# Toytiny/CMFlow

Hardware: AMD Instinct MI355X
Metric: frame-pairs/sec CMFlow fwd+bwd (higher is better)
Workload: dtype f32; 1 GPU; cmflow fwd+bwd training (7 cross-modal losses + Adam, train-mode BN) step, N=256, B=64 per GPU (global 64), ball-query r=2/4/8/16 K=4/8/16/32, kNN K=8; synthetic clouds, seeded random-init weights; parallelism=dp1

## Files before the change

cmflow_amd/csrc/gemm.hip:

```cpp
#include <algorithm>
#include <atomic>
#include <cstdlib>
#include <cstring>
#include <type_traits>
#include "cmf_common.h"
#include "../../include/cmflow_hip.h"

typedef float f32x16 __attribute__((ext_vector_type(16)));

constexpr int G_THREADS = 256;
#ifndef CMF_GEMM_BK
#define CMF_GEMM_BK 16
#endif
constexpr int G_BK = CMF_GEMM_BK;
constexpr int G_KT = G_BK / 4;
constexpr int G_RP = 256 / G_KT;
constexpr int G_LDS_LD = G_BK + 4;

#include "gemm_args.h"
#ifdef CMF_GEMM_DIAG
#define GDIAG(p) ((p).diag)
#else
#define GDIAG(p) 0
#endif
// ... 45 lines not shown
}

template <int BM, int BN, bool A_T, bool B_T, int EPI = 0, int GMODE = 0>
__global__ __launch_bounds__(G_THREADS, (BM > 128 || BN > 128) ? 2 : 3) void gemm_kernel(const GemmArgs p)
{
    constexpr bool GATHER = GMODE == 1, GATHER_B = GMODE == 2, GATHER_Z = GMODE == 3 || GMODE == 4, GATHER_S = GMODE == 4;
    static_assert(!GATHER_Z || (!A_T && !B_T && EPI == 4 && (BM == 128 || (BM == 256 && GMODE == 4)) && BN == 128), "gathered Z rows: the kind-4 data gradient");
    static_assert(!GATHER || (!A_T && B_T), "gathering A operand: A[M][K] W[N][K] layout");
    static_assert(!GATHER_B || (A_T && !B_T), "gathering B operand: A[K][M] B[K][N] layout");
    constexpr int WARPS_M = (BM == 64) ? 2 : ((BN >= 128) ? 2 : 4);
    constexpr int WARPS_N = 4 / WARPS_M;
    constexpr int WM = BM / WARPS_M, WN = BN / WARPS_N;
    constexpr int TM = WM / 32, TN = WN / 32;
    static_assert(TM >= 1 && TN >= 1, "tile");
    constexpr int A_LD = A_T ? BM + 4 : G_LDS_LD, A_SZ = A_T ? G_BK * (BM + 4) : BM * G_LDS_LD;
    constexpr int B_LD = B_T ? G_LDS_LD : BN + 4, B_SZ = B_T ? BN * G_LDS_LD : G_BK * (BN + 4);
    extern __shared__ __attribute__((aligned(16))) float smem[];
    float *As = smem;
    float *Bs = smem + 2 * A_SZ;

    const int tiles_m = (p.M + BM - 1) / BM, tiles_n = (p.N + BN - 1) / BN;
    int tm, tn, split;
    {
        const int id = blockIdx.x, nx = 8;
        const int xcd = id % nx, slot = id / nx;
        if (p.split_k > 1) {
            const int tiles = tiles_m * tiles_n;
            split = xcd + nx * (slot / tiles);
            const int t = slot % tiles;
            tm = t / tiles_n; tn = t % tiles_n;
            if (split >= p.split_k) return;
        } else {
            const int per = (tiles_m + nx - 1) / nx;
            split = 0;
            tm = xcd * per + slot / tiles_n;
            tn = slot % tiles_n;
            if (tm >= tiles_m || slot / tiles_n >= per) return;
        }
    }
    const unsigned long long t_start = p.trace ? wall_clock64() : 0ull;
    const int kchunks_total = (p.K + G_BK - 1) / G_BK;
    const int kchunks_per = (kchunks_total + p.split_k - 1) / p.split_k;
    const int kc_begin = split * kchunks_per;
    const int kc_end = min(kchunks_total, kc_begin + kchunks_per);
    const int m0 = tm * BM, n0 = tn * BN;
    const int tid = threadIdx.x, lane = tid & 63, wid = __builtin_amdgcn_readfirstlane(tid >> 6);
    const int wm = wid / WARPS_N, wn = wid % WARPS_N;

    constexpr int A_TPR = BM / 4, A_RPI = G_THREADS / A_TPR;
    constexpr int B_TPR = BN / 4, B_RPI = G_THREADS / B_TPR;
    constexpr int A_IT = A_T ? (G_BK / A_RPI) : (BM / G_RP);
    constexpr int B_IT = B_T ? (BN / G_RP) : (G_BK / B_RPI);
    float4 ra[A_IT], rb[B_IT];
    int gbrow[GATHER_B ? B_IT : 1];
    float4 gbd[GATHER_B ? B_IT : 1], gbw[3];
    float4 rz[A_T ? A_IT : 1];
    const bool bnbA = A_T && p.bnb_z != nullptr;
    float bal[4] = {1.f, 1.f, 1.f, 1.f}, bbe[4] = {0.f, 0.f, 0.f, 0.f}, bga[4] = {0.f, 0.f, 0.f, 0.f}, bmu[4] = {0.f, 0.f, 0.f, 0.f};
    int k0_loaded = 0;
    const int bnb_writers = tiles_n < G_BK ? tiles_n : G_BK;
    if (A_T && bnbA) {
        const int m = m0 + (tid % A_TPR) * 4;
#pragma unroll
        for (int j = 0; j < 4; ++j) {
            bmu[j] = p.bnb_mean[m + j];
            cmf_bnb_coef(p.bnb_a[m + j], bmu[j], p.bnb_invstd[m + j], p.bnb_sums[m + j], p.bnb_sums[p.M + m + j], p.bnb_ic,
                         bal[j], bbe[j], bga[j]);
        }
    }
    float4 psa = make_float4(1.f, 1.f, 1.f, 1.f), psc = make_float4(0.f, 0.f, 0.f, 0.f);
    float4 qsa = make_float4(1.f, 1.f, 1.f, 1.f), qsc = make_float4(0.f, 0.f, 0.f, 0.f);
    unsigned kmask = 0xF;
    const bool proA = !A_T && p.pro_a != nullptr;
    const bool proB = !B_T && p.prob_a != nullptr;
    const bool edge_mn = (m0 + BM > p.M) || (n0 + BN > p.N);
    if (proB) {
        const int n = n0 + (tid % B_TPR) * 4;
        float t[8] = {1, 1, 1, 1, 0, 0, 0, 0};
        for (int j = 0; j < 4; ++j) if (n + j < p.N) { t[j] = p.prob_a[n + j]; t[4 + j] = p.prob_c[n + j]; }
        qsa = make_float4(t[0], t[1], t[2], t[3]); qsc = make_float4(t[4], t[5], t[6], t[7]);
    }

    auto load_tiles = [&](int kc) {
        const int k0 = kc * G_BK;
        const bool fast = !edge_mn && (k0 + G_BK <= p.K);
        k0_loaded = k0;
        if (fast) {
            if (!A_T) {
                const int kk = k0 + (tid % G_KT) * 4;
                if (proA) { psa = *(const float4 *)(p.pro_a + kk); psc = *(const float4 *)(p.pro_c + kk); }
                const float *src = p.A + (long long)(m0 + (tid / G_KT)) * p.lda + kk;
#pragma unroll
                for (int i = 0; i < A_IT; ++i) ra[i] = *(const float4 *)(src + (long long)G_RP * i * p.lda);
            } else {
                const float *src = p.A + (long long)(k0 + tid / A_TPR) * p.lda + m0 + (tid % A_TPR) * 4;
#pragma unroll
                for (int i = 0; i < A_IT; ++i) ra[i] = *(const float4 *)(src + (long long)A_RPI * i * p.lda);
                if (bnbA) {
                    const float *zs = p.bnb_z + (long long)(k0 + tid / A_TPR) * p.ldbz + m0 + (tid % A_TPR) * 4;
#pragma unroll
                    for (int i = 0; i < A_IT; ++i) rz[A_T ? i : 0] = *(const float4 *)(zs + (long long)A_RPI * i * p.ldbz);
                }
            }
            if (B_T) {
                const float *src = p.B + (long long)(n0 + (tid / G_KT)) * p.ldb + k0 + (tid % G_KT) * 4;
#pragma unroll
                for (int i = 0; i < B_IT; ++i) rb[i] = *(const float4 *)(src + (long long)G_RP * i * p.ldb);
            } else if (GATHER_B) {
#pragma unroll
                for (int i = 0; i < B_IT; ++i) {
                    const int k = k0 + tid / B_TPR + B_RPI * i;
                    rb[GATHER_B ? i : 0] = *(const float4 *)(p.B + (long long)gbrow[GATHER_B ? i : 0] * p.ldb + n0 + (tid % B_TPR) * 4);
                    gbd[GATHER_B ? i : 0] = *(const float4 *)(p.ga_dxyz + (long long)k * 4);
                    gbrow[GATHER_B ? i : 0] = k + G_BK < p.K ? p.ga_rows[k + G_BK] : 0;
                }
            } else {
                const float *src = p.B + (long long)(k0 + tid / B_TPR) * p.ldb + n0 + (tid % B_TPR) * 4;
#pragma unroll
                for (int i = 0; i < B_IT; ++i) rb[i] = *(const float4 *)(src + (long long)B_RPI * i * p.ldb);
            }
            kmask = 0xF;
            return;
        }
        if (GATHER_B) __builtin_trap();
        auto ld4 = [&](const float *src, int valid) {
            float t[4] = {0.f, 0.f, 0.f, 0.f};
            if (valid >= 4) return *(const float4 *)src;
            for (int j = 0; j < 4; ++j) if (j < valid) t[j] = src[j];
            return make_float4(t[0], t[1], t[2], t[3]);
        };
        if (!A_T) {
            const int kk = k0 + (tid % G_KT) * 4;
            const int kv = max(0, min(4, p.K - kk));
            kmask = (1u << kv) - 1u;
            if (proA) { psa = ld4(p.pro_a + kk, kv); psc = ld4(p.pro_c + kk, kv); }
#pragma unroll
            for (int i = 0; i < A_IT; ++i) {
                const int m = m0 + (tid / G_KT) + G_RP * i;
                ra[i] = (m < p.M && kv > 0) ? ld4(p.A + (long long)m * p.lda + kk, kv) : make_float4(0.f, 0.f, 0.f, 0.f);
                if (m >= p.M) ra[i].x = __builtin_nanf("");
            }
        } else {
#pragma unroll
            for (int i = 0; i < A_IT; ++i) {
                const int k = k0 + tid / A_TPR + A_RPI * i, m = m0 + (tid % A_TPR) * 4;
                ra[i] = (k < p.K && m < p.M) ? ld4(p.A + (long long)k * p.lda + m, p.M - m) : make_float4(0.f, 0.f, 0.f, 0.f);
            }
        }
        if (B_T) {
            const int kk = k0 + (tid % G_KT) * 4;
            const int kv = max(0, min(4, p.K - kk));
#pragma unroll
            for (int i = 0; i < B_IT; ++i) {
                const int n = n0 + (tid / G_KT) + G_RP * i;
                rb[i] = (n < p.N && kv > 0) ? ld4(p.B + (long long)n * p.ldb + kk, kv) : make_float4(0.f, 0.f, 0.f, 0.f);
            }
        } else {
#pragma unroll
            for (int i = 0; i < B_IT; ++i) {
                const int k = k0 + tid / B_TPR + B_RPI * i, n = n0 + (tid % B_TPR) * 4;
                rb[i] = (k < p.K && n < p.N) ? ld4(p.B + (long long)k * p.ldb + n, p.N - n) : make_float4(0.f, 0.f, 0.f, 0.f);
                if (!(k < p.K)) rb[i].x = __builtin_nanf("");
            }
        }
    };
    auto pro4 = [&](float4 v, const float4 &sa, const float4 &sc) {
        v.x = fmaxf(fmaf(sa.x, v.x, sc.x), 0.f); v.y = fmaxf(fmaf(sa.y, v.y, sc.y), 0.f);
        v.z = fmaxf(fmaf(sa.z, v.z, sc.z), 0.f); v.w = fmaxf(fmaf(sa.w, v.w, sc.w), 0.f);
        return v;
    };
    auto store_A = [&](int buf) {
        float *dst = As + buf * A_SZ;
        if (!A_T) {
#pragma unroll
            for (int i = 0; i < A_IT; ++i) {
                float4 v = ra[i];
                if (proA) {
                    const bool dead = v.x != v.x;
                    v = pro4(v, psa, psc);
                    if (dead) v = make_float4(0.f, 0.f, 0.f, 0.f);
                    if (kmask != 0xF) { if (!(kmask & 1)) v.x = 0.f; if (!(kmask & 2)) v.y = 0.f;
                                        if (!(kmask & 4)) v.z = 0.f; if (!(kmask & 8)) v.w = 0.f; }
                } else if (v.x != v.x && edge_mn) v = make_float4(0.f, 0.f, 0.f, 0.f);
                *(float4 *)(dst + ((tid / G_KT) + G_RP * i) * G_LDS_LD + (tid % G_KT) * 4) = v;
            }
        } else {
#pragma unroll
            for (int i = 0; i < A_IT; ++i) {
                const int k = tid / A_TPR + A_RPI * i, m = (tid % A_TPR) * 4;
                float4 v = ra[i];
                if (bnbA) {
                    const float4 zz = rz[A_T ? i : 0];
                    v.x = cmf_bnb_apply(v.x, zz.x, bmu[0], bal[0], bbe[0], bga[0]); v.y = cmf_bnb_apply(v.y, zz.y, bmu[1], bal[1], bbe[1], bga[1]);
                    v.z = cmf_bnb_apply(v.z, zz.z, bmu[2], bal[2], bbe[2], bga[2]); v.w = cmf_bnb_apply(v.w, zz.w, bmu[3], bal[3], bbe[3], bga[3]);
                    if (p.bnb_out && (k % bnb_writers) == tn) *(float4 *)(p.bnb_out + (long long)(k0_loaded + k) * p.ldbo + m0 + m) = v;
                }
                *(float4 *)(dst + k * A_LD + m) = v;
            }
        }
    };
    auto store_B = [&](int buf) {
        float *dst = Bs + buf * B_SZ;
        if (B_T) {
#pragma unroll
            for (int i = 0; i < B_IT; ++i)
                *(float4 *)(dst + ((tid / G_KT) + G_RP * i) * G_LDS_LD + (tid % G_KT) * 4) = rb[i];
        } else {
#pragma unroll
            for (int i = 0; i < B_IT; ++i) {
                const int k = tid / B_TPR + B_RPI * i, n = (tid % B_TPR) * 4;
                float4 v = rb[i];
                if (GATHER_B) {
                    const float4 d = gbd[GATHER_B ? i : 0];
                    v.x += fmaf(gbw[2].x, d.z, fmaf(gbw[1].x, d.y, gbw[0].x * d.x)); v.y += fmaf(gbw[2].y, d.z, fmaf(gbw[1].y, d.y, gbw[0].y * d.x));
                    v.z += fmaf(gbw[2].z, d.z, fmaf(gbw[1].z, d.y, gbw[0].z * d.x)); v.w += fmaf(gbw[2].w, d.z, fmaf(gbw[1].w, d.y, gbw[0].w * d.x));
                }
                if (proB) {
                    const bool dead = v.x != v.x;
                    v = pro4(v, qsa, qsc);
                    if (dead) v = make_float4(0.f, 0.f, 0.f, 0.f);
                } else if (v.x != v.x) v = make_float4(0.f, 0.f, 0.f, 0.f);
                *(float4 *)(dst + k * B_LD + n) = v;
            }
        }
    };

    f32x16 acc[TM][TN];
#pragma unroll
    for (int i = 0; i < TM; ++i)
#pragma unroll
        for (int j = 0; j < TN; ++j)
#pragma unroll
            for (int r = 0; r < 16; ++r) acc[i][j][r] = 0.f;

    constexpr int D_ASLOTS = BM * (G_BK / 4), D_BSLOTS = BN * (G_BK / 4);
    constexpr int D_ANI = D_ASLOTS / G_THREADS, D_BNI = D_BSLOTS / G_THREADS;
    constexpr int D_STAGE = (D_ASLOTS + D_BSLOTS) * 4 + (GATHER ? 96 : 32);
    const bool direct = G_BK == 16 && !edge_mn && (p.K % G_BK == 0) && !p.no_direct && !bnbA && !GATHER_B;
    if (GATHER_B) {
#pragma unroll
        for (int i = 0; i < B_IT; ++i) gbrow[GATHER_B ? i : 0] = p.ga_rows[kc_begin * G_BK + tid / B_TPR + B_RPI * i];
#pragma unroll
        for (int c = 0; c < 3; ++c) gbw[c] = *(const float4 *)(p.ga_wx + (long long)c * p.N + n0 + (tid % B_TPR) * 4);
    }
    if (direct && kc_begin < kc_end) {
        const long long pro_delta = proA ? (long long)(p.pro_c - p.pro_a) : 0ll;
        if (GATHER && !proA) __builtin_trap();
        long long asrc[D_ANI];
        const float *gconst = nullptr;
        if (GATHER) {
#pragma unroll
            for (int q = 0; q < D_ANI; ++q) asrc[q] = (long long)p.ga_rows[m0 + (((q * 4 + wid) * 64 + lane) >> 2)] * p.lda;
            if (!(B_T && BN > 128)) gconst = (lane < 4 ? p.pro_a : lane < 8 ? p.pro_c : p.ga_wx + (long long)((lane >> 2) - 2) * p.K) + 4 * (lane & 3);
        }
        if (GATHER_S) {
#pragma unroll
            for (int q = 0; q < D_ANI; ++q) asrc[q] = (long long)p.ga_arows[m0 + (((q * 4 + wid) * 64 + lane) >> 2)] * p.lda;
        }
        constexpr bool WIDE_B = GATHER && B_T && BN > 128;
        __amdgpu_buffer_rsrc_t rB = __builtin_amdgcn_make_buffer_rsrc((void *)(p.B + (long long)n0 * p.ldb), 0, -1, 0x00020000);
        const unsigned offB = (unsigned)((((wid * 64 + lane) >> 2) * (int)p.ldb + 4 * ((lane & 3) ^ g_swz((wid * 64 + lane) >> 2))) * 4);
        auto issue = [&](int kc, int st) {
            const int k0 = kc * G_BK;
            float *sa = smem + st * D_STAGE, *sb = sa + D_ASLOTS * 4, *sp = sb + D_BSLOTS * 4;
#pragma unroll
            for (int q = 0; q < D_ANI; ++q) {
                const int grp = q * 4 + wid, sl = grp * 64 + lane;
                const float *g;
                if (!A_T) { const int row = sl >> 2; g = p.A + ((GATHER || GATHER_S) ? asrc[q] : (long long)(m0 + row) * p.lda) + k0 + 4 * ((sl & 3) ^ g_swz(row)); }
                else { const int k = sl / (BM / 4); g = p.A + (long long)(k0 + k) * p.lda + m0 + 4 * ((sl % (BM / 4)) ^ (((k >> 2) & 1) * 8)); }
                __builtin_amdgcn_global_load_lds((g_gptr)g, (g_lptr)(sa + grp * 256), 16, 0, 0);
            }
#pragma unroll
            for (int q = 0; q < D_BNI; ++q) {
                const int grp = q * 4 + wid, sl = grp * 64 + lane;
                if (WIDE_B) {
                    __builtin_amdgcn_raw_ptr_buffer_load_lds(rB, (g_lptr)(sb + grp * 256), 16, offB, (unsigned)((q * 64 * (int)p.ldb + k0) * 4), 0, 0);
                    continue;
                }
                const float *g;
                if (B_T) { const int row = sl >> 2; g = p.B + (long long)(n0 + row) * p.ldb + k0 + 4 * ((sl & 3) ^ g_swz(row)); }
                else { const int k = sl / (BN / 4); g = p.B + (long long)(k0 + k) * p.ldb + n0 + 4 * ((sl % (BN / 4)) ^ (((k >> 2) & 1) * 8)); }
                __builtin_amdgcn_global_load_lds((g_gptr)g, (g_lptr)(sb + grp * 256), 16, 0, 0);
            }
            if (GATHER) {
                if (WIDE_B) {
                    int l = lane;
                    asm volatile("" : "+v"(l));
                    if (wid == 0 && l < 20) {
                        const float *gc = (l < 4 ? p.pro_a : l < 8 ? p.pro_c : p.ga_wx + (long long)((l >> 2) - 2) * p.K) + 4 * (l & 3);
                        __builtin_amdgcn_global_load_lds((g_gptr)(gc + k0), (g_lptr)sp, 16, 0, 0);
                    }
                } else
                if (wid == 0 && lane < 20) __builtin_amdgcn_global_load_lds((g_gptr)(gconst + k0), (g_lptr)sp, 16, 0, 0);
            } else
            if (proA && wid == 0 && lane < 8)
                __builtin_amdgcn_global_load_lds((g_gptr)(p.pro_a + (lane < 4 ? 0ll : pro_delta) + k0 + 4 * (lane & 3)), (g_lptr)sp, 16, 0, 0);
        };
        auto wait_prev = [&](bool newest_outstanding) {
            if (!newest_outstanding) { CMF_WAIT_VMCNT(0); return; }
            if (proA && wid == 0) { CMF_WAIT_VMCNT(D_ANI + D_BNI + 1); } else { CMF_WAIT_VMCNT(D_ANI + D_BNI); }
        };
        const int nch = kc_end - kc_begin;
        issue(kc_begin, 0);
        if (nch > 1) issue(kc_begin + 1, 1);
        wait_prev(nch > 1);
        __builtin_amdgcn_s_barrier();
        const int frow = lane & 31, h = lane >> 5;
        int arow[TM], aswz[TM], brow[TN], bswz[TN];
#pragma unroll
        for (int i = 0; i < TM; ++i) { arow[i] = wm * WM + i * 32 + frow; aswz[i] = g_swz(arow[i]); }
#pragma unroll
        for (int j = 0; j < TN; ++j) { brow[j] = wn * WN + j * 32 + frow; bswz[j] = g_swz(brow[j]); }
        float qa[TN], qc[TN];
#pragma unroll
        for (int j = 0; j < TN; ++j) {
            const int n = n0 + brow[j];
            qa[j] = (proB && n < p.N) ? p.prob_a[n] : 1.f; qc[j] = (proB && n < p.N) ? p.prob_c[n] : 0.f;
        }
        f32x4 af[2][TM], bf[2][TN], pa4[2], pc4[2];
        f32x4 gw0, gw1, gw2, gdq[TM];
        if (GATHER) {
#pragma unroll
            for (int i = 0; i < TM; ++i) gdq[i] = *(const f32x4 *)(p.ga_dxyz + (long long)(m0 + arow[i]) * 4);
        }
        auto read_frags = [&](const float *sa, const float *sb, const float *sp, int k8, int w) {
            const int kq = k8 / 4 + h;
#pragma unroll
            for (int i = 0; i < TM; ++i) {
                if (!A_T) af[w][i] = g_lds_read128(g_lds_addr(sa + (arow[i] * 4 + (kq ^ aswz[i])) * 4));
                else {
                    const unsigned q = g_lds_addr(sa + (4 * kq) * BM + ((((arow[i] >> 2) ^ (h * 8)) << 2) | (arow[i] & 3)));
                    af[w][i].x = g_lds_read32<0>(q); af[w][i].y = g_lds_read32<BM * 4>(q);
                    af[w][i].z = g_lds_read32<BM * 8>(q); af[w][i].w = g_lds_read32<BM * 12>(q);
                }
            }
#pragma unroll
            for (int j = 0; j < TN; ++j) {
                if (B_T) bf[w][j] = g_lds_read128(g_lds_addr(sb + (brow[j] * 4 + (kq ^ bswz[j])) * 4));
                else {
                    const unsigned q = g_lds_addr(sb + (4 * kq) * BN + ((((brow[j] >> 2) ^ (h * 8)) << 2) | (brow[j] & 3)));
                    bf[w][j].x = g_lds_read32<0>(q); bf[w][j].y = g_lds_read32<BN * 4>(q);
                    bf[w][j].z = g_lds_read32<BN * 8>(q); bf[w][j].w = g_lds_read32<BN * 12>(q);
                }
            }
            if (GATHER) {
                pa4[0] = g_lds_read128(g_lds_addr(sp + 4 * kq)); pc4[0] = g_lds_read128(g_lds_addr(sp + 16 + 4 * kq));
                gw0 = g_lds_read128(g_lds_addr(sp + 32 + 4 * kq)); gw1 = g_lds_read128(g_lds_addr(sp + 48 + 4 * kq));
                gw2 = g_lds_read128(g_lds_addr(sp + 64 + 4 * kq));
            } else
            if (proA) { pa4[w] = g_lds_read128(g_lds_addr(sp + 4 * kq)); pc4[w] = g_lds_read128(g_lds_addr(sp + 16 + 4 * kq)); }
        };
        auto pin_frags = [&](int w) {
#pragma unroll
            for (int i = 0; i < TM; ++i) g_pin(af[w][i]);
#pragma unroll
            for (int j = 0; j < TN; ++j) g_pin(bf[w][j]);
            if (GATHER) { g_pin(pa4[0]); g_pin(pc4[0]); g_pin(gw0); g_pin(gw1); g_pin(gw2); }
            else if (proA) { g_pin(pa4[w]); g_pin(pc4[w]); }
        };
        auto gather_prologue = [&](int w) {
#pragma unroll
            for (int i = 0; i < TM; ++i) {
                const float dx = gdq[i].x, dy = gdq[i].y, dz = gdq[i].z;
                f32x4 z = af[w][i];
                z.x += fmaf(gw2.x, dz, fmaf(gw1.x, dy, gw0.x * dx)); z.y += fmaf(gw2.y, dz, fmaf(gw1.y, dy, gw0.y * dx));
                z.z += fmaf(gw2.z, dz, fmaf(gw1.z, dy, gw0.z * dx)); z.w += fmaf(gw2.w, dz, fmaf(gw1.w, dy, gw0.w * dx));
                af[w][i].x = fmaxf(fmaf(pa4[0].x, z.x, pc4[0].x), 0.f); af[w][i].y = fmaxf(fmaf(pa4[0].y, z.y, pc4[0].y), 0.f);
                af[w][i].z = fmaxf(fmaf(pa4[0].z, z.z, pc4[0].z), 0.f); af[w][i].w = fmaxf(fmaf(pa4[0].w, z.w, pc4[0].w), 0.f);
            }
        };
        auto prologue_step = [&](int w) {
            if (!GATHER && proA) {
#pragma unroll
                for (int i = 0; i < TM; ++i) {
                    af[w][i].x = fmaxf(fmaf(pa4[w].x, af[w][i].x, pc4[w].x), 0.f); af[w][i].y = fmaxf(fmaf(pa4[w].y, af[w][i].y, pc4[w].y), 0.f);
                    af[w][i].z = fmaxf(fmaf(pa4[w].z, af[w][i].z, pc4[w].z), 0.f); af[w][i].w = fmaxf(fmaf(pa4[w].w, af[w][i].w, pc4[w].w), 0.f);
                }
            }
            if (proB) {
#pragma unroll
                for (int j = 0; j < TN; ++j) {
                    bf[w][j].x = fmaxf(fmaf(qa[j], bf[w][j].x, qc[j]), 0.f); bf[w][j].y = fmaxf(fmaf(qa[j], bf[w][j].y, qc[j]), 0.f);
                    bf[w][j].z = fmaxf(fmaf(qa[j], bf[w][j].z, qc[j]), 0.f); bf[w][j].w = fmaxf(fmaf(qa[j], bf[w][j].w, qc[j]), 0.f);
                }
            }
        };
        auto mfma_step = [&](int w) {
            prologue_step(w);
#pragma unroll
            for (int i = 0; i < TM; ++i)
#pragma unroll
                for (int j = 0; j < TN; ++j) {
                    acc[i][j] = __builtin_amdgcn_mfma_f32_32x32x2f32(af[w][i].x, bf[w][j].x, acc[i][j], 0, 0, 0);
                    acc[i][j] = __builtin_amdgcn_mfma_f32_32x32x2f32(af[w][i].y, bf[w][j].y, acc[i][j], 0, 0, 0);
                    acc[i][j] = __builtin_amdgcn_mfma_f32_32x32x2f32(af[w][i].z, bf[w][j].z, acc[i][j], 0, 0, 0);
                    acc[i][j] = __builtin_amdgcn_mfma_f32_32x32x2f32(af[w][i].w, bf[w][j].w, acc[i][j], 0, 0, 0);
                }
        };
        int st = 0;
#ifndef CMF_NO_SETPRIO
        __builtin_amdgcn_s_setprio(1);
#endif
        {
            {
                const float *sa = smem, *sb = sa + D_ASLOTS * 4, *sp = sb + D_BSLOTS * 4;
                read_frags(sa, sb, sp, 0, 0);
                g_lds_wait(); pin_frags(0);
                if (GATHER) gather_prologue(0);
            }
            for (int c = 0; c < nch; ++c) {
                {
                    const float *sa = smem + st * D_STAGE, *sb = sa + D_ASLOTS * 4, *sp = sb + D_BSLOTS * 4;
                    read_frags(sa, sb, sp, 8, 1);
                }
                mfma_step(0);
                g_lds_wait(); pin_frags(1);
                if (GATHER) gather_prologue(1);
                if (c + 2 < nch && !(GDIAG(p) & 1)) issue(kc_begin + c + 2, st == 0 ? 2 : st - 1);
                const int sn = st == 2 ? 0 : st + 1;
                const float *sa = smem + sn * D_STAGE, *sb = sa + D_ASLOTS * 4, *sp = sb + D_BSLOTS * 4;
                if (c + 1 < nch) {
                    if (!(GDIAG(p) & 3)) wait_prev(c + 2 < nch);
                    if (!(GDIAG(p) & 4)) __builtin_amdgcn_s_barrier();
                    read_frags(sa, sb, sp, 0, 0);
                }
                mfma_step(1);
                if (c + 1 < nch) { g_lds_wait(); pin_frags(0); if (GATHER) gather_prologue(0); }
                st = sn;
            }
            __builtin_amdgcn_s_barrier();
        }
        __builtin_amdgcn_s_setprio(0);
    } else
    if (GATHER || GATHER_S) __builtin_trap();
    else
    if (kc_begin < kc_end) {
        load_tiles(kc_begin);
        store_A(0); store_B(0);
        __syncthreads();
        int buf = 0;
        const int frow = lane & 31, fk = (lane >> 5) * 4;
        for (int kc = kc_begin; kc < kc_end; ++kc) {
            const bool more = kc + 1 < kc_end;
            if (more) load_tiles(kc + 1);
            const float *a_s = As + buf * A_SZ + (A_T ? fk * A_LD + wm * WM + frow : (wm * WM + frow) * A_LD + fk);
            const float *b_s = Bs + buf * B_SZ + (B_T ? (wn * WN + frow) * B_LD + fk : fk * B_LD + wn * WN + frow);
#pragma unroll
            for (int k8 = 0; k8 < G_BK; k8 += 8) {
                float4 af[TM], bf[TN];
#pragma unroll
                for (int i = 0; i < TM; ++i) {
                    if (!A_T) af[i] = *(const float4 *)(a_s + i * 32 * A_LD + k8);
                    else { const float *q = a_s + k8 * A_LD + i * 32;
                           af[i] = make_float4(q[0], q[A_LD], q[2 * A_LD], q[3 * A_LD]); }
                }
#pragma unroll
                for (int j = 0; j < TN; ++j) {
                    if (B_T) bf[j] = *(const float4 *)(b_s + j * 32 * B_LD + k8);
                    else { const float *q = b_s + k8 * B_LD + j * 32;
                           bf[j] = make_float4(q[0], q[B_LD], q[2 * B_LD], q[3 * B_LD]); }
                }
#pragma unroll
                for (int i = 0; i < TM; ++i)
#pragma unroll
                    for (int j = 0; j < TN; ++j) {
                        acc[i][j] = __builtin_amdgcn_mfma_f32_32x32x2f32(af[i].x, bf[j].x, acc[i][j], 0, 0, 0);
                        acc[i][j] = __builtin_amdgcn_mfma_f32_32x32x2f32(af[i].y, bf[j].y, acc[i][j], 0, 0, 0);
                        acc[i][j] = __builtin_amdgcn_mfma_f32_32x32x2f32(af[i].z, bf[j].z, acc[i][j], 0, 0, 0);
                        acc[i][j] = __builtin_amdgcn_mfma_f32_32x32x2f32(af[i].w, bf[j].w, acc[i][j], 0, 0, 0);
                    }
                if (k8 == (G_BK >= 32 ? G_BK - 16 : G_BK - 8) && more) { store_A(buf ^ 1); store_B(buf ^ 1); }
            }
            asm volatile("s_waitcnt lgkmcnt(0)" ::: "memory");
            __builtin_amdgcn_s_barrier();
            asm volatile("" ::: "memory");
            buf ^= 1;
        }
    }

    const unsigned long long t_main = p.trace ? wall_clock64() : 0ull;
    unsigned long long t_e[3] = {0ull, 0ull, 0ull};
    if (GDIAG(p) & 8) {
#pragma unroll
        for (int i = 0; i < TM; ++i)
#pragma unroll
            for (int j = 0; j < TN; ++j) g_keep(acc[i][j]);
        return;
    }
    constexpr int T_LD = BN + 4;
// ... 772 lines not shown
extern "C" int cmf_gemm_profile_sampling(int every)
{
    CMF_CHECK_ARG(every >= 1);
    std::lock_guard<std::mutex> lock(g_gprof.mu);
    g_gprof.sample_every = every;
    return 0;
}

extern "C" int cmf_gemm_profile_eligible(long long *launches, double *flops)
{
    std::lock_guard<std::mutex> lock(g_gprof.mu);
    if (launches) *launches = g_gprof.launches_eligible;
    if (flops) *flops = g_gprof.flops_eligible;
    return 0;
}

extern "C" int cmf_gemm_profile_end(long long *launches_timed, double *ms_timed, double *flops_timed, long long *launches_all,
                                    double *flops_all)
{
    std::lock_guard<std::mutex> lock(g_gprof.mu);
    g_gprof.on = false;
    if (hipDeviceSynchronize() != hipSuccess) return (int)hipGetLastError();
    double ms = 0.0;
    for (size_t i = 0; i < g_gprof.used; ++i) {
        float t = 0.f;
        if (hipEventElapsedTime(&t, g_gprof.events[2 * i], g_gprof.events[2 * i + 1]) != hipSuccess) return (int)hipGetLastError();
        ms += t;
        g_gprof.recs[i].ms = t;
    }
    if (launches_timed) *launches_timed = (long long)g_gprof.used;
    if (ms_timed) *ms_timed = ms;
    if (flops_timed) *flops_timed = g_gprof.flops_timed;
    if (launches_all) *launches_all = g_gprof.launches_all;
    if (flops_all) *flops_all = g_gprof.flops_all;
    return 0;
}

extern "C" long long cmf_gemm_profile_records(cmf_gemm_launch_record *out, long long max_records)
{
    std::lock_guard<std::mutex> lock(g_gprof.mu);
    const long long n = (long long)g_gprof.used < max_records ? (long long)g_gprof.used : max_records;
    for (long long i = 0; i < n && out; ++i) out[i] = g_gprof.recs[(size_t)i];
    return (long long)g_gprof.used;
}

template <int BM, int BN, bool A_T, bool B_T, int EPI = 0, int GMODE = 0>
static int launch(const GemmArgs &a, hipStream_t st)
{
    constexpr bool GATHER = GMODE == 1;
    const int tiles_m = (a.M + BM - 1) / BM, tiles_n = (a.N + BN - 1) / BN;
    const int per = (tiles_m + 7) / 8;
    dim3 grid(a.split_k > 1 ? 8 * ((a.split_k + 7) / 8) * tiles_m * tiles_n : 8 * per * tiles_n);
    const size_t lds_reg = (size_t)2 * ((A_T ? G_BK * (BM + 4) : BM * G_LDS_LD) + (B_T ? BN * G_LDS_LD : G_BK * (BN + 4))) * sizeof(float);
    const size_t lds_dir = (size_t)G_STAGES * ((BM + BN) * (G_BK / 4) * 4 + (GATHER ? 96 : 32)) * sizeof(float);
    const size_t lds = lds_reg > lds_dir ? lds_reg : lds_dir;
    static std::atomic<unsigned> set_mask[4];
    int dev = 0;
    (void)hipGetDevice(&dev);
    const unsigned bit = 1u << (dev & 31);
    if (dev >= 128 || !(set_mask[dev >> 5].load(std::memory_order_acquire) & bit)) {
        if (hipFuncSetAttribute((const void *)gemm_kernel<BM, BN, A_T, B_T, EPI, GMODE>, hipFuncAttributeMaxDynamicSharedMemorySize,
                                (int)lds) != hipSuccess) return (int)hipGetLastError();
        if (dev < 128) set_mask[dev >> 5].fetch_or(bit, std::memory_order_release);
    }
    const long long pe = gprof_open(2.0 * a.M * a.N * a.K, st, &a, (A_T ? 2 : 0) | (B_T ? 1 : 0), BM, BN);
    if (unsigned long long *tb = trace_take(grid.x, st)) {
        GemmArgs t = a;
        t.trace = tb;
        hipLaunchKernelGGL((gemm_kernel<BM, BN, A_T, B_T, EPI, GMODE>), grid, dim3(G_THREADS), lds, st, t);
        gprof_close(pe, st);
        return cmf_launch_status();
    }
    hipLaunchKernelGGL((gemm_kernel<BM, BN, A_T, B_T, EPI, GMODE>), grid, dim3(G_THREADS), lds, st, a);
    gprof_close(pe, st);
    return cmf_launch_status();
}

static int gemm_diag_rt()
{
    static const int v = getenv("CMF_GEMM_DIAG_RT") ? atoi(getenv("CMF_GEMM_DIAG_RT")) : 0;
    return v;
}

static bool gemm_tall()
{
    static const bool on = cmf_env_on("CMF_GEMM_TALL");
    return on;
}

static bool gemm_wide()
{
    static const bool on = cmf_env_on("CMF_GEMM_WIDE");
    return on;
}

extern "C" int cmf_gemm(int M, int N, int K, int a_t, int b_t,
                        const float *A, long long lda, const float *B, long long ldb, float *C, long long ldc,
                        const float *pro_a, const float *pro_c, const float *prob_a, const float *prob_c,
                        const float *bias, int act, float *stats,
                        int bwd_mode, const float *Z, long long ldz,
                        const float *ea, const float *ec, const float *emean, const float *einvstd,
                        const float *dxyz, int split_k, float *workspace, int accumulate, void *stream)
{
    CMF_CHECK_ARG(M >= 0 && N >= 0 && K >= 0 && split_k >= 1);
    if (M == 0 || N == 0) return 0;
    CMF_CHECK_ARG(A && B && C);
    CMF_CHECK_ARG(!(a_t && pro_a));
// ... 82 lines not shown
    g.stats = stats; g.bwd_mode = 1; g.Z = Y; g.ldz = ldy; g.ea = ea; g.ec = ec; g.emean = emean; g.einvstd = einvstd; g.dxyz = dxyz;
    g.ga_rows = rows; g.ga_dxyz = dxyz; g.ga_wx = wx3; g.split_k = 1;
    g.diag = gemm_diag_rt();
    return launch<128, 128, false, false, 4, 3>(g, st);
}

static thread_local long long g_dxsum_points_hint = 0;
void cmf_gemm_dx_gather_sum_hint(long long points) { g_dxsum_points_hint = points; }

extern "C" int cmf_gemm_dx_gather_sum(int M, int cin, int cout, const float *dZ, long long ldz, const float *W, long long ldw,
                                      const float *Y, long long ldy, const int *arows, const int *pts, const float *dxyz2,
                                      const float *wx3, const float *ea, const float *ec, const float *emean, const float *einvstd,
                                      float *pieces, float *stats, void *stream)
{
    CMF_CHECK_ARG(M > 0 && cin > 0 && cout > 0 && M % 128 == 0 && cin % 128 == 0 && cout % G_BK == 0);
    CMF_CHECK_ARG(dZ && W && Y && arows && pts && dxyz2 && wx3 && ea && ec && emean && einvstd && pieces && stats);
    CMF_CHECK_ARG(ldz % 4 == 0 && ldw % 4 == 0 && ldy % 4 == 0);
    CMF_CHECK_ARG((((uintptr_t)dZ | (uintptr_t)W | (uintptr_t)Y | (uintptr_t)dxyz2) & 15) == 0);
    hipStream_t st = (hipStream_t)stream;
    GemmArgs g{};
    g.M = M; g.N = cin; g.K = cout; g.A = dZ; g.lda = ldz; g.B = W; g.ldb = ldw; g.C = pieces; g.ldc = cin;
    g.stats = stats; g.bwd_mode = 1; g.Z = Y; g.ldz = ldy; g.ea = ea; g.ec = ec; g.emean = emean; g.einvstd = einvstd; g.dxyz = dxyz2;
    g.ga_rows = pts; g.ga_dxyz = dxyz2; g.ga_wx = wx3; g.ga_arows = arows; g.ga_pieces = pieces; g.split_k = 1;
    const long long npts = g_dxsum_points_hint > 0 ? g_dxsum_points_hint : (long long)M;
    g.ga_y32 = (npts * ldy + cin) * 4 < (1ll << 32) ? 1 : 0;
    g_dxsum_points_hint = 0;
    g.diag = gemm_diag_rt();
    return launch<128, 128, false, false, 4, 4>(g, st);
}

extern "C" int cmf_gemm_dw_gather_split(int cout, int cin, long long nrows)
{
    if (!gemm_tall() || cout <= 0 || cin <= 0 || cout % 256 || cin % 128 || nrows % G_BK) return 0;
    const long long tiles = (long long)(cout / 256) * (cin / 128), chunks = nrows / G_BK;
    int s = (int)(512 / tiles) / 8 * 8;
    while (s >= 8 && chunks / s < 8) s -= 8;
    return s >= 16 ? s : 0;
}

extern "C" int cmf_gemm_dw_gather(int cout, int cin, long long nrows, const float *dZ, long long ldz, const float *Y, long long ldy,
                                  const int *rows, const float *dxyz, const float *wx3, const float *prob_a, const float *prob_c,
                                  float *dW, long long lddw, int split_k, float *workspace, int accumulate, void *stream)
{
    CMF_CHECK_ARG(cout > 0 && cin > 0 && nrows > 0 && nrows < (1ll << 31) && split_k >= 1);
    CMF_CHECK_ARG(cout % 128 == 0 && cin % 128 == 0 && nrows % G_BK == 0);
    CMF_CHECK_ARG(dZ && Y && rows && dxyz && wx3 && prob_a && prob_c && dW && (split_k == 1 || workspace));
    CMF_CHECK_ARG(ldz % 4 == 0 && ldy % 4 == 0 && lddw % 4 == 0);
    CMF_CHECK_ARG((((uintptr_t)dZ | (uintptr_t)Y | (uintptr_t)dxyz | (uintptr_t)wx3 | (uintptr_t)dW) & 15) == 0);
    hipStream_t st = (hipStream_t)stream;
    GemmArgs g{};
    g.M = cout; g.N = cin; g.K = (int)nrows; g.A = dZ; g.lda = ldz; g.B = Y; g.ldb = ldy;
    g.C = split_k > 1 ? workspace : dW; g.ldc = split_k > 1 ? cin : lddw;
    g.prob_a = prob_a; g.prob_c = prob_c; g.split_k = split_k; g.accumulate = split_k > 1 ? 0 : accumulate;
    g.ga_rows = rows; g.ga_dxyz = dxyz; g.ga_wx = wx3; g.no_direct = 1;
    const bool tall = split_k > 1 && split_k == cmf_gemm_dw_gather_split(cout, cin, nrows);
    const int err = tall ? launch<256, 128, true, false, 0, 2>(g, st) : launch<128, 128, true, false, 0, 2>(g, st);
    if (err) return err;
    if (split_k > 1) return cmf_splitk_reduce(cout, cin, split_k, workspace, dW, lddw, accumulate, st);
    return 0;
}

extern "C" int cmf_gemm_dw_gather_bn_bwd(int cout, int cin, long long nrows, const float *dU, long long ldu, const float *Z, long long ldz,
                                         const float *a, const float *mean, const float *invstd, const float *sums, float *dZ_out, long long ldo,
                                         const float *Y, long long ldy, const int *rows, const float *dxyz, const float *wx3,
                                         const float *prob_a, const float *prob_c, float *dW, long long lddw, int split_k, float *workspace,
                                         int accumulate, void *stream)
{
    CMF_CHECK_ARG(cout > 0 && cin > 0 && nrows > 0 && nrows < (1ll << 31) && split_k >= 1);
    CMF_CHECK_ARG(cout % 128 == 0 && cin % 128 == 0 && nrows % G_BK == 0);
    CMF_CHECK_ARG(dU && Z && a && mean && invstd && sums && dZ_out && dZ_out != dU && Y && rows && dxyz && wx3 && prob_a && prob_c && dW && (split_k == 1 || workspace));
    CMF_CHECK_ARG(ldu % 4 == 0 && ldz % 4 == 0 && ldo % 4 == 0 && ldy % 4 == 0 && lddw % 4 == 0);
    CMF_CHECK_ARG((((uintptr_t)dU | (uintptr_t)Z | (uintptr_t)dZ_out | (uintptr_t)Y | (uintptr_t)dxyz | (uintptr_t)wx3 | (uintptr_t)dW) & 15) == 0);
    hipStream_t st = (hipStream_t)stream;
    GemmArgs g{};
    g.M = cout; g.N = cin; g.K = (int)nrows; g.A = dU; g.lda = ldu; g.B = Y; g.ldb = ldy;
    g.C = split_k > 1 ? workspace : dW; g.ldc = split_k > 1 ? cin : lddw;
    g.prob_a = prob_a; g.prob_c = prob_c; g.split_k = split_k; g.accumulate = split_k > 1 ? 0 : accumulate;
    g.ga_rows = rows; g.ga_dxyz = dxyz; g.ga_wx = wx3; g.no_direct = 1;
    g.bnb_z = Z; g.ldbz = ldz; g.bnb_a = a; g.bnb_mean = mean; g.bnb_invstd = invstd; g.bnb_sums = sums;
    g.bnb_ic = (float)(1.0 / (double)nrows); g.bnb_out = dZ_out; g.ldbo = ldo;
    const bool tall = split_k > 1 && split_k == cmf_gemm_dw_gather_split(cout, cin, nrows);
    const int err = tall ? launch<256, 128, true, false, 0, 2>(g, st) : launch<128, 128, true, false, 0, 2>(g, st);
    if (err) return err;
    if (split_k > 1) return cmf_splitk_reduce(cout, cin, split_k, workspace, dW, lddw, accumulate, st);
    return 0;
}

extern "C" int cmf_gemm_tiles_m(int M) { return M > 64 ? (M + 127) / 128 : 1; }
```

Measured before the change: 3412 frame-pairs/s.

## Route gather-B weight-gradient GEMMs through direct-to-LDS pipelined path with in-LDS transform

The gather-B dW GEMM variants (with and without fused BN backward) previously forced the register-staged load path via no_direct. They now use a triple-buffered global_load_lds pipeline. Gathered rows, dxyz offsets and per-column constants are staged in LDS, and the gather add, prologue ReLU and BN-backward apply run in place on the LDS tiles between MFMA steps. The aim is to overlap the irregular gather loads with compute and drop the register round-trip. In exchange it adds extra LDS footprint, inline asm waits and complex vmcnt bookkeeping.

```diff
diff --git a/cmflow_amd/csrc/gemm.hip b/cmflow_amd/csrc/gemm.hip
--- a/cmflow_amd/csrc/gemm.hip
+++ b/cmflow_amd/csrc/gemm.hip
@@ -121,15 +121,13 @@
     constexpr int A_IT = A_T ? (G_BK / A_RPI) : (BM / G_RP);
     constexpr int B_IT = B_T ? (BN / G_RP) : (G_BK / B_RPI);
     float4 ra[A_IT], rb[B_IT];
-    int gbrow[GATHER_B ? B_IT : 1];
-    float4 gbd[GATHER_B ? B_IT : 1], gbw[3];
-    float4 rz[A_T ? A_IT : 1];
-    const bool bnbA = A_T && p.bnb_z != nullptr;
+    const int dt_ca = ((lane % (BM / 4)) ^ ((wid & 1) * 8)) * 4, dt_cb = ((lane & 31) ^ ((wid & 1) * 8)) * 4;
+    const bool bnbA = GATHER_B && p.bnb_z != nullptr;
     float bal[4] = {1.f, 1.f, 1.f, 1.f}, bbe[4] = {0.f, 0.f, 0.f, 0.f}, bga[4] = {0.f, 0.f, 0.f, 0.f}, bmu[4] = {0.f, 0.f, 0.f, 0.f};
-    int k0_loaded = 0;
     const int bnb_writers = tiles_n < G_BK ? tiles_n : G_BK;
-    if (A_T && bnbA) {
-        const int m = m0 + (tid % A_TPR) * 4;
+    constexpr bool DT_LDS_A = BM > 128;
+    if (bnbA && !DT_LDS_A) {
+        const int m = m0 + dt_ca;
 #pragma unroll
         for (int j = 0; j < 4; ++j) {
             bmu[j] = p.bnb_mean[m + j];
@@ -143,7 +141,7 @@
     const bool proA = !A_T && p.pro_a != nullptr;
     const bool proB = !B_T && p.prob_a != nullptr;
     const bool edge_mn = (m0 + BM > p.M) || (n0 + BN > p.N);
-    if (proB) {
+    if (proB && !GATHER_B) {
         const int n = n0 + (tid % B_TPR) * 4;
         float t[8] = {1, 1, 1, 1, 0, 0, 0, 0};
         for (int j = 0; j < 4; ++j) if (n + j < p.N) { t[j] = p.prob_a[n + j]; t[4 + j] = p.prob_c[n + j]; }
@@ -153,7 +151,6 @@
     auto load_tiles = [&](int kc) {
         const int k0 = kc * G_BK;
         const bool fast = !edge_mn && (k0 + G_BK <= p.K);
-        k0_loaded = k0;
         if (fast) {
             if (!A_T) {
                 const int kk = k0 + (tid % G_KT) * 4;
@@ -165,24 +162,11 @@
                 const float *src = p.A + (long long)(k0 + tid / A_TPR) * p.lda + m0 + (tid % A_TPR) * 4;
 #pragma unroll
                 for (int i = 0; i < A_IT; ++i) ra[i] = *(const float4 *)(src + (long long)A_RPI * i * p.lda);
-                if (bnbA) {
-                    const float *zs = p.bnb_z + (long long)(k0 + tid / A_TPR) * p.ldbz + m0 + (tid % A_TPR) * 4;
-#pragma unroll
-                    for (int i = 0; i < A_IT; ++i) rz[A_T ? i : 0] = *(const float4 *)(zs + (long long)A_RPI * i * p.ldbz);
-                }
             }
             if (B_T) {
                 const float *src = p.B + (long long)(n0 + (tid / G_KT)) * p.ldb + k0 + (tid % G_KT) * 4;
 #pragma unroll
                 for (int i = 0; i < B_IT; ++i) rb[i] = *(const float4 *)(src + (long long)G_RP * i * p.ldb);
-            } else if (GATHER_B) {
-#pragma unroll
-                for (int i = 0; i < B_IT; ++i) {
-                    const int k = k0 + tid / B_TPR + B_RPI * i;
-                    rb[GATHER_B ? i : 0] = *(const float4 *)(p.B + (long long)gbrow[GATHER_B ? i : 0] * p.ldb + n0 + (tid % B_TPR) * 4);
-                    gbd[GATHER_B ? i : 0] = *(const float4 *)(p.ga_dxyz + (long long)k * 4);
-                    gbrow[GATHER_B ? i : 0] = k + G_BK < p.K ? p.ga_rows[k + G_BK] : 0;
-                }
             } else {
                 const float *src = p.B + (long long)(k0 + tid / B_TPR) * p.ldb + n0 + (tid % B_TPR) * 4;
 #pragma unroll
@@ -191,7 +175,6 @@
             kmask = 0xF;
             return;
         }
-        if (GATHER_B) __builtin_trap();
         auto ld4 = [&](const float *src, int valid) {
             float t[4] = {0.f, 0.f, 0.f, 0.f};
             if (valid >= 4) return *(const float4 *)src;
@@ -257,14 +240,7 @@
 #pragma unroll
             for (int i = 0; i < A_IT; ++i) {
                 const int k = tid / A_TPR + A_RPI * i, m = (tid % A_TPR) * 4;
-                float4 v = ra[i];
-                if (bnbA) {
-                    const float4 zz = rz[A_T ? i : 0];
-                    v.x = cmf_bnb_apply(v.x, zz.x, bmu[0], bal[0], bbe[0], bga[0]); v.y = cmf_bnb_apply(v.y, zz.y, bmu[1], bal[1], bbe[1], bga[1]);
-                    v.z = cmf_bnb_apply(v.z, zz.z, bmu[2], bal[2], bbe[2], bga[2]); v.w = cmf_bnb_apply(v.w, zz.w, bmu[3], bal[3], bbe[3], bga[3]);
-                    if (p.bnb_out && (k % bnb_writers) == tn) *(float4 *)(p.bnb_out + (long long)(k0_loaded + k) * p.ldbo + m0 + m) = v;
-                }
-                *(float4 *)(dst + k * A_LD + m) = v;
+                *(float4 *)(dst + k * A_LD + m) = ra[i];
             }
         }
     };
@@ -279,11 +255,6 @@
             for (int i = 0; i < B_IT; ++i) {
                 const int k = tid / B_TPR + B_RPI * i, n = (tid % B_TPR) * 4;
                 float4 v = rb[i];
-                if (GATHER_B) {
-                    const float4 d = gbd[GATHER_B ? i : 0];
-                    v.x += fmaf(gbw[2].x, d.z, fmaf(gbw[1].x, d.y, gbw[0].x * d.x)); v.y += fmaf(gbw[2].y, d.z, fmaf(gbw[1].y, d.y, gbw[0].y * d.x));
-                    v.z += fmaf(gbw[2].z, d.z, fmaf(gbw[1].z, d.y, gbw[0].z * d.x)); v.w += fmaf(gbw[2].w, d.z, fmaf(gbw[1].w, d.y, gbw[0].w * d.x));
-                }
                 if (proB) {
                     const bool dead = v.x != v.x;
                     v = pro4(v, qsa, qsc);
@@ -304,14 +275,8 @@
 
     constexpr int D_ASLOTS = BM * (G_BK / 4), D_BSLOTS = BN * (G_BK / 4);
     constexpr int D_ANI = D_ASLOTS / G_THREADS, D_BNI = D_BSLOTS / G_THREADS;
-    constexpr int D_STAGE = (D_ASLOTS + D_BSLOTS) * 4 + (GATHER ? 96 : 32);
-    const bool direct = G_BK == 16 && !edge_mn && (p.K % G_BK == 0) && !p.no_direct && !bnbA && !GATHER_B;
-    if (GATHER_B) {
-#pragma unroll
-        for (int i = 0; i < B_IT; ++i) gbrow[GATHER_B ? i : 0] = p.ga_rows[kc_begin * G_BK + tid / B_TPR + B_RPI * i];
-#pragma unroll
-        for (int c = 0; c < 3; ++c) gbw[c] = *(const float4 *)(p.ga_wx + (long long)c * p.N + n0 + (tid % B_TPR) * 4);
-    }
+    constexpr int D_STAGE = (D_ASLOTS + D_BSLOTS) * 4 + ((GATHER || GATHER_B) ? 96 : 32);
+    const bool direct = G_BK == 16 && !edge_mn && (p.K % G_BK == 0) && (GATHER_B || !p.no_direct);
     if (direct && kc_begin < kc_end) {
         const long long pro_delta = proA ? (long long)(p.pro_c - p.pro_a) : 0ll;
         if (GATHER && !proA) __builtin_trap();
@@ -371,10 +336,12 @@
             if (proA && wid == 0) { CMF_WAIT_VMCNT(D_ANI + D_BNI + 1); } else { CMF_WAIT_VMCNT(D_ANI + D_BNI); }
         };
         const int nch = kc_end - kc_begin;
-        issue(kc_begin, 0);
-        if (nch > 1) issue(kc_begin + 1, 1);
-        wait_prev(nch > 1);
-        __builtin_amdgcn_s_barrier();
+        if constexpr (!GATHER_B) {
+            issue(kc_begin, 0);
+            if (nch > 1) issue(kc_begin + 1, 1);
+            wait_prev(nch > 1);
+            __builtin_amdgcn_s_barrier();
+        }
         const int frow = lane & 31, h = lane >> 5;
         int arow[TM], aswz[TM], brow[TN], bswz[TN];
 #pragma unroll
@@ -447,7 +414,7 @@
                     af[w][i].z = fmaxf(fmaf(pa4[w].z, af[w][i].z, pc4[w].z), 0.f); af[w][i].w = fmaxf(fmaf(pa4[w].w, af[w][i].w, pc4[w].w), 0.f);
                 }
             }
-            if (proB) {
+            if (proB && !GATHER_B) {
 #pragma unroll
                 for (int j = 0; j < TN; ++j) {
                     bf[w][j].x = fmaxf(fmaf(qa[j], bf[w][j].x, qc[j]), 0.f); bf[w][j].y = fmaxf(fmaf(qa[j], bf[w][j].y, qc[j]), 0.f);
@@ -471,6 +438,148 @@
 #ifndef CMF_NO_SETPRIO
         __builtin_amdgcn_s_setprio(1);
 #endif
+        if constexpr (GATHER_B) {
+            static_assert(BN == 128 && G_BK == 16 && (BM == 128 || BM == 256), "direct-transform loop: 4 k-rows of both operands per wave");
+            constexpr int SA = BM / 4, KA = 64 / SA;
+            constexpr int NL = D_ANI + D_BNI + 2;
+            const int ka = 4 * wid + lane / SA, kb = 4 * wid + (lane >> 5);
+            unsigned wmask = 0;
+#pragma unroll
+            for (int q = 0; q < D_ANI; ++q) if (bnbA && p.bnb_out && ((ka + KA * q) % bnb_writers) == tn) wmask |= 1u << q;
+            f32x4 rz[D_ANI];
+            float *cstB = smem + G_STAGES * D_STAGE, *cstA = cstB + 5 * BN;
+            if (tid < BN) {
+                const int n = n0 + tid;
+                cstB[tid] = p.ga_wx[n]; cstB[BN + tid] = p.ga_wx[(long long)p.N + n]; cstB[2 * BN + tid] = p.ga_wx[2ll * p.N + n];
+                cstB[3 * BN + tid] = proB ? p.prob_a[n] : 1.f; cstB[4 * BN + tid] = proB ? p.prob_c[n] : 0.f;
+            }
+            if (DT_LDS_A && bnbA && tid < BM) {
+                const int m = m0 + tid;
+                float al, be, ga;
+                const float mu = p.bnb_mean[m];
+                cmf_bnb_coef(p.bnb_a[m], mu, p.bnb_invstd[m], p.bnb_sums[m], p.bnb_sums[p.M + m], p.bnb_ic, al, be, ga);
+                cstA[tid] = al; cstA[BM + tid] = be; cstA[2 * BM + tid] = ga; cstA[3 * BM + tid] = mu;
+            }
+            __syncthreads();
+            auto issue_t = [&](int kc, int stg, const int (&brow)[D_BNI]) {
+                const int k0 = kc * G_BK;
+                float *sa = smem + stg * D_STAGE, *sb = sa + D_ASLOTS * 4, *sp = sb + D_BSLOTS * 4 + wid * 20;
+#pragma unroll
+                for (int q = 0; q < D_ANI; ++q)
+                    __builtin_amdgcn_global_load_lds((g_gptr)(p.A + (long long)(k0 + ka + KA * q) * p.lda + m0 + dt_ca), (g_lptr)(sa + (wid * D_ANI + q) * 256), 16, 0, 0);
+#pragma unroll
+                for (int q = 0; q < D_BNI; ++q)
+                    __builtin_amdgcn_global_load_lds((g_gptr)(p.B + (long long)brow[q] * p.ldb + n0 + dt_cb), (g_lptr)(sb + (wid * D_BNI + q) * 256), 16, 0, 0);
+                if (lane < 4) {
+                    const int kr = k0 + 2 * G_BK + 4 * wid + lane;
+                    __builtin_amdgcn_global_load_lds((g_gptr)(p.ga_rows + (kr < p.K ? kr : 0)), (g_lptr)sp, 4, 0, 0);
+                    __builtin_amdgcn_global_load_lds((g_gptr)(p.ga_dxyz + (long long)(k0 + 4 * wid + lane) * 4), (g_lptr)(sp + 4), 16, 0, 0);
+                }
+            };
+            auto load_z = [&](int kc) {
+#pragma unroll
+                for (int q = 0; q < D_ANI; ++q) {
+                    const float *zs = p.bnb_z + (long long)(kc * G_BK + ka + KA * q) * p.ldbz + m0 + dt_ca;
+                    asm volatile("global_load_dwordx4 %0, %1, off" : "=&v"(rz[q]) : "v"(zs) : "memory");
+                }
+            };
+            auto wait_t = [&](bool newest_outstanding) {
+                if (newest_outstanding) { CMF_WAIT_VMCNT(NL); } else { CMF_WAIT_VMCNT(0); }
+            };
+            auto lds_write128 = [&](unsigned addr, const f32x4 &v) { asm volatile("ds_write_b128 %0, %1" :: "v"(addr), "v"(v) : "memory"); };
+            auto transform = [&](int kc, int stg) {
+                float *sa = smem + stg * D_STAGE, *sb = sa + D_ASLOTS * 4, *sp = sb + D_BSLOTS * 4 + wid * 20;
+                const unsigned aa = g_lds_addr(sa + wid * D_ANI * 256 + lane * 4), ab = g_lds_addr(sb + wid * D_BNI * 256 + lane * 4);
+                f32x4 vb[D_BNI], d[D_BNI], va[D_ANI], gbw[3], qsa, qsc, cA[4];
+#pragma unroll
+                for (int q = 0; q < D_BNI; ++q) { vb[q] = g_lds_read128(ab + q * 1024); d[q] = g_lds_read128(g_lds_addr(sp + 4 + ((lane >> 5) + 2 * q) * 4)); }
+#pragma unroll
+                for (int c = 0; c < 3; ++c) gbw[c] = g_lds_read128(g_lds_addr(cstB + c * BN + dt_cb));
+                qsa = g_lds_read128(g_lds_addr(cstB + 3 * BN + dt_cb)); qsc = g_lds_read128(g_lds_addr(cstB + 4 * BN + dt_cb));
+                g_lds_wait();
+                g_pin(gbw[0]); g_pin(gbw[1]); g_pin(gbw[2]); g_pin(qsa); g_pin(qsc);
+#pragma unroll
+                for (int q = 0; q < D_BNI; ++q) {
+                    g_pin(vb[q]); g_pin(d[q]);
+                    f32x4 v = vb[q];
+                    v.x += fmaf(gbw[2].x, d[q].z, fmaf(gbw[1].x, d[q].y, gbw[0].x * d[q].x)); v.y += fmaf(gbw[2].y, d[q].z, fmaf(gbw[1].y, d[q].y, gbw[0].y * d[q].x));
+                    v.z += fmaf(gbw[2].z, d[q].z, fmaf(gbw[1].z, d[q].y, gbw[0].z * d[q].x)); v.w += fmaf(gbw[2].w, d[q].z, fmaf(gbw[1].w, d[q].y, gbw[0].w * d[q].x));
+                    if (proB) {
+                        const bool dead = v.x != v.x;
+                        v.x = fmaxf(fmaf(qsa.x, v.x, qsc.x), 0.f); v.y = fmaxf(fmaf(qsa.y, v.y, qsc.y), 0.f);
+                        v.z = fmaxf(fmaf(qsa.z, v.z, qsc.z), 0.f); v.w = fmaxf(fmaf(qsa.w, v.w, qsc.w), 0.f);
+                        if (dead) v = f32x4{0.f, 0.f, 0.f, 0.f};
+                    } else if (v.x != v.x) v = f32x4{0.f, 0.f, 0.f, 0.f};
+                    lds_write128(ab + q * 1024, v);
+                }
+                if (bnbA) {
+#pragma unroll
+                    for (int q = 0; q < D_ANI; ++q) va[q] = g_lds_read128(aa + q * 1024);
+                    if (DT_LDS_A) {
+#pragma unroll
+                        for (int c = 0; c < 4; ++c) cA[c] = g_lds_read128(g_lds_addr(cstA + c * BM + dt_ca));
+                    }
+                    g_lds_wait();
+                    if (DT_LDS_A) {
+                        g_pin(cA[0]); g_pin(cA[1]); g_pin(cA[2]); g_pin(cA[3]);
+#pragma unroll
+                        for (int j = 0; j < 4; ++j) { bal[j] = cA[0][j]; bbe[j] = cA[1][j]; bga[j] = cA[2][j]; bmu[j] = cA[3][j]; }
+                    }
+#pragma unroll
+                    for (int q = 0; q < D_ANI; ++q) {
+                        g_pin(va[q]); g_pin(rz[q]);
+                        f32x4 v = va[q];
+                        const f32x4 zz = rz[q];
+                        v.x = cmf_bnb_apply(v.x, zz.x, bmu[0], bal[0], bbe[0], bga[0]); v.y = cmf_bnb_apply(v.y, zz.y, bmu[1], bal[1], bbe[1], bga[1]);
+                        v.z = cmf_bnb_apply(v.z, zz.z, bmu[2], bal[2], bbe[2], bga[2]); v.w = cmf_bnb_apply(v.w, zz.w, bmu[3], bal[3], bbe[3], bga[3]);
+                        lds_write128(aa + q * 1024, v);
+                        if (wmask & (1u << q)) *(f32x4 *)(p.bnb_out + (long long)(kc * G_BK + ka + KA * q) * p.ldbo + m0 + dt_ca) = v;
+                    }
+                }
+            };
+            {
+                int br0[D_BNI], br1[D_BNI];
+#pragma unroll
+                for (int q = 0; q < D_BNI; ++q) {
+                    br0[q] = p.ga_rows[kc_begin * G_BK + kb + 2 * q];
+                    br1[q] = nch > 1 ? p.ga_rows[(kc_begin + 1) * G_BK + kb + 2 * q] : 0;
+                }
+                issue_t(kc_begin, 0, br0);
+                if (bnbA) load_z(kc_begin);
+                if (nch > 1) issue_t(kc_begin + 1, 1, br1);
+                wait_t(nch > 1);
+                transform(kc_begin, 0);
+            }
+            for (int c = 0; c < nch; ++c) {
+                const int sn = st == 2 ? 0 : st + 1;
+                if (bnbA && c + 1 < nch) load_z(kc_begin + c + 1);
+                g_lds_wait();
+                __builtin_amdgcn_s_barrier();
+                const float *sa = smem + st * D_STAGE, *sb = sa + D_ASLOTS * 4, *sp = sb + D_BSLOTS * 4;
+                read_frags(sa, sb, sp, 0, 0);
+                if (c > 0) mfma_step(1);
+                g_lds_wait(); pin_frags(0);
+                read_frags(sa, sb, sp, 8, 1);
+                int br[D_BNI];
+                f32x4 brv = {0.f, 0.f, 0.f, 0.f};
+                if (c + 2 < nch) brv = g_lds_read128(g_lds_addr(sp + wid * 20));
+                mfma_step(0);
+                g_lds_wait(); pin_frags(1); g_pin(brv);
+                if (c + 2 < nch) {
+#pragma unroll
+                    for (int q = 0; q < D_BNI; ++q) {
+                        const float f = (lane >> 5) ? (q ? brv.w : brv.y) : (q ? brv.z : brv.x);
+                        br[q] = __builtin_bit_cast(int, f);
+                    }
+                    issue_t(kc_begin + c + 2, st == 0 ? 2 : st - 1, br);
+                }
+                if (c + 1 < nch) { wait_t(c + 2 < nch); transform(kc_begin + c + 1, sn); }
+                st = sn;
+            }
+            mfma_step(1);
+            g_lds_wait();
+            __builtin_amdgcn_s_barrier();
+        } else
         {
             {
                 const float *sa = smem, *sb = sa + D_ASLOTS * 4, *sp = sb + D_BSLOTS * 4;
@@ -502,9 +611,8 @@
         }
         __builtin_amdgcn_s_setprio(0);
     } else
-    if (GATHER || GATHER_S) __builtin_trap();
-    else
     if (kc_begin < kc_end) {
+        if (GATHER || GATHER_S || GATHER_B) __builtin_trap();
         load_tiles(kc_begin);
         store_A(0); store_B(0);
         __syncthreads();
@@ -1383,7 +1491,8 @@
     const int per = (tiles_m + 7) / 8;
     dim3 grid(a.split_k > 1 ? 8 * ((a.split_k + 7) / 8) * tiles_m * tiles_n : 8 * per * tiles_n);
     const size_t lds_reg = (size_t)2 * ((A_T ? G_BK * (BM + 4) : BM * G_LDS_LD) + (B_T ? BN * G_LDS_LD : G_BK * (BN + 4))) * sizeof(float);
-    const size_t lds_dir = (size_t)G_STAGES * ((BM + BN) * (G_BK / 4) * 4 + (GATHER ? 96 : 32)) * sizeof(float);
+    const size_t lds_dir = (size_t)G_STAGES * ((BM + BN) * (G_BK / 4) * 4 + ((GATHER || GMODE == 2) ? 96 : 32)) * sizeof(float) +
+                           (GMODE == 2 ? (size_t)(5 * BN + (BM > 128 ? 4 * BM : 0)) * sizeof(float) : 0);
     const size_t lds = lds_reg > lds_dir ? lds_reg : lds_dir;
     static std::atomic<unsigned> set_mask[4];
     int dev = 0;
@@ -1572,7 +1681,7 @@
     g.M = cout; g.N = cin; g.K = (int)nrows; g.A = dZ; g.lda = ldz; g.B = Y; g.ldb = ldy;
     g.C = split_k > 1 ? workspace : dW; g.ldc = split_k > 1 ? cin : lddw;
     g.prob_a = prob_a; g.prob_c = prob_c; g.split_k = split_k; g.accumulate = split_k > 1 ? 0 : accumulate;
-    g.ga_rows = rows; g.ga_dxyz = dxyz; g.ga_wx = wx3; g.no_direct = 1;
+    g.ga_rows = rows; g.ga_dxyz = dxyz; g.ga_wx = wx3;
     const bool tall = split_k > 1 && split_k == cmf_gemm_dw_gather_split(cout, cin, nrows);
     const int err = tall ? launch<256, 128, true, false, 0, 2>(g, st) : launch<128, 128, true, false, 0, 2>(g, st);
     if (err) return err;
@@ -1596,7 +1705,7 @@
     g.M = cout; g.N = cin; g.K = (int)nrows; g.A = dU; g.lda = ldu; g.B = Y; g.ldb = ldy;
     g.C = split_k > 1 ? workspace : dW; g.ldc = split_k > 1 ? cin : lddw;
     g.prob_a = prob_a; g.prob_c = prob_c; g.split_k = split_k; g.accumulate = split_k > 1 ? 0 : accumulate;
-    g.ga_rows = rows; g.ga_dxyz = dxyz; g.ga_wx = wx3; g.no_direct = 1;
+    g.ga_rows = rows; g.ga_dxyz = dxyz; g.ga_wx = wx3;
     g.bnb_z = Z; g.ldbz = ldz; g.bnb_a = a; g.bnb_mean = mean; g.bnb_invstd = invstd; g.bnb_sums = sums;
     g.bnb_ic = (float)(1.0 / (double)nrows); g.bnb_out = dZ_out; g.ldbo = ldo;
     const bool tall = split_k > 1 && split_k == cmf_gemm_dw_gather_split(cout, cin, nrows);
```

Result: no change. 3382 frame-pairs/s (-0.9%).
